# qdrant/qdrant

Hardware: AMD Instinct MI355X
Metric: QPS @ recall@10, brute-force, d=768 10M vecs, f32 cosine top-10 (higher is better)
Workload: dtype f32 (int8 prefilter + exact f32 re-score)

## Files before the change

### qdrant_amd/csrc/api_core.hip

```cpp
#include "api_internal.hpp"

namespace qmx {

static thread_local std::string g_last_error;
const std::string &last_error_text() { return g_last_error; }

void set_error(const char *fmt, ...) {
    char buf[1024];
    va_list ap;
    va_start(ap, fmt);
    vsnprintf(buf, sizeof(buf), fmt, ap);
    va_end(ap);
    g_last_error = buf;
}

int32_t hip_status(hipError_t e, const char *what, const char *file, int line) {
    set_error("HIP error %d (%s) at %s:%d: %s", (int)e, hipGetErrorString(e), file, line, what);
    (void)hipGetLastError();
    switch (e) {
        case hipErrorOutOfMemory: return QMX_ERR_OUT_OF_MEMORY;
        case hipErrorNoDevice:
        case hipErrorInvalidDevice:
        case hipErrorNoBinaryForGpu:
        case hipErrorInsufficientDriver: return QMX_ERR_NO_DEVICE;
        case hipErrorNotReady: return QMX_ERR_NOT_READY;
        case hipErrorInvalidValue: return QMX_ERR_BAD_ARG;
        default: return QMX_ERR_OTHER;
    }
}

static const char *const g_option_names[OPT_COUNT] = {"no_mfma_scan", "no_mfma16", "no_prescan", "prescan_shift", "hnsw_log_cap", "no_split_scan", "split_min_queries", "no_split256", "no_pq_pair", "no_pq_prefilter", "pq_prefilter_min_queries", "hnsw_pq_per_cu", "tq_rotate_block", "no_topk_small", "verify_max_per_query", "hnsw_pq_direct_walk", "hnsw_pq_table_build", "hnsw_no_pq_prefilter", "hnsw_no_lds_visited", "pq_lut_no_lds", "hnsw_per_cu", "hnsw_reference_heap_order", "tq_wide_min_queries", "tq_wide_high_digit", "sq_wide_min_queries", "i8_resident", "group_matrix_bytes", "debug"};
struct OptionTable {
    std::atomic<int64_t> v[OPT_COUNT];
    int64_t initial[OPT_COUNT];
    OptionTable() {
        for (int i = 0; i < OPT_COUNT; ++i) {
            char env[64] = "QMX_";
            size_t k = 4;
            for (const char *c = g_option_names[i]; *c && k + 1 < sizeof(env); ++c) env[k++] = (char)toupper((unsigned char)*c);
            env[k] = 0;
            const char *e = getenv(env);
            int64_t val = 0;
            if (e) { val = (*e >= '0' && *e <= '9') ? atoll(e) : 1; }
            if (i == OPT_PRESCAN_SHIFT && !e) val = 10;
            if (i == OPT_SPLIT_MIN_QUERIES && !e) val = 1;
            if (i == OPT_PQ_PREFILTER_MIN_QUERIES && !e) val = 4;
            if (i == OPT_TQ_WIDE_MIN_QUERIES && !e) val = 33;
            if (i == OPT_SQ_WIDE_MIN_QUERIES && !e) val = 33;
            if (i == OPT_I8_RESIDENT && !e) val = 1;
            initial[i] = val;
            v[i].store(val, std::memory_order_relaxed);
        }
    }
};
static OptionTable g_options;
int64_t option(Option o) { return g_options.v[o].load(std::memory_order_relaxed); }

static thread_local const void *g_last_kernel = nullptr;
const void *last_noted_kernel() { return g_last_kernel; }
void note_kernel(const void *host_function) { g_last_kernel = host_function; }

void clear_stale_error() {
    hipError_t e = hipGetLastError();
    if (e != hipSuccess) {
        const bool debug = option(OPT_DEBUG) != 0;
        if (debug) fprintf(stderr, "[qmx] dropped stale HIP error %d (%s) before a kernel launch\n", (int)e, hipGetErrorString(e));
    }
}

bool is_device_ptr(const void *p) {
    if (!p) return false;
    hipPointerAttribute_t attr;
    hipError_t e = hipPointerGetAttributes(&attr, p);
    if (e != hipSuccess) {
        (void)hipGetLastError();
        return false;
    }
    return attr.type == hipMemoryTypeDevice || attr.type == hipMemoryTypeManaged;
}

uint32_t elem_bytes(uint32_t dtype) {
    switch (dtype) {
        case QMX_DTYPE_F32: return 4;
        case QMX_DTYPE_F16: return 2;
        default: return 1;
    }
}



int32_t check_device(int32_t device_id, hipDeviceProp_t *prop_out) {
    int count = 0;
    hipError_t e = hipGetDeviceCount(&count);
    if (e != hipSuccess || count == 0) {
        (void)hipGetLastError();
        set_error("no HIP device visible (%s); libqdrant_amd has no CPU fallback", e == hipSuccess ? "count=0" : hipGetErrorString(e));
        return QMX_ERR_NO_DEVICE;
    }
    QMX_REQUIRE(device_id >= 0 && device_id < count, QMX_ERR_NO_DEVICE, "device %d out of range (have %d)", device_id, count);
    hipDeviceProp_t prop;
    QMX_HIP(hipGetDeviceProperties(&prop, device_id));
    QMX_REQUIRE(strncmp(prop.gcnArchName, "gfx950", 6) == 0, QMX_ERR_NO_DEVICE,
                "device %d is %s; this library ships gfx950 (MI355X) code objects only", device_id, prop.gcnArchName);
    QMX_HIP(hipSetDevice(device_id));
    if (prop_out) *prop_out = prop;
    return QMX_OK;
}

}


extern "C" {


uint32_t qmx_abi_version(void) { return 8; }

static int option_index(const char *name) {
    if (!name) return -1;
    for (int i = 0; i < OPT_COUNT; ++i)
        if (strcmp(name, g_option_names[i]) == 0) return i;
    return -1;
}
int32_t qmx_set_option(const char *name, int64_t value) {
    const int i = option_index(name);
    QMX_REQUIRE(i >= 0, QMX_ERR_BAD_ARG, "unknown option '%s'", name ? name : "(null)");
    g_options.v[i].store(value < 0 ? g_options.initial[i] : value, std::memory_order_relaxed);
    return QMX_OK;
}
int32_t qmx_get_option(const char *name, int64_t *out_value) {
    const int i = option_index(name);
    QMX_REQUIRE(i >= 0 && out_value, QMX_ERR_BAD_ARG, "unknown option '%s'", name ? name : "(null)");
    *out_value = option((Option)i);
// ... 30 lines not shown
```

### qdrant_amd/csrc/api_search.hip

```cpp
#include "api_internal.hpp"

extern "C" {

struct SearchCall {
    qmx_query *q;
    uint32_t top;
    const uint32_t *d_ids;
    uint64_t n_cand;
    qmx_scored_point *d_out;
    uint32_t *d_counts;
    const volatile uint8_t *is_stopped;
    qmx_counters *counters;
    bool timed;
    uint32_t launches;
};

static ScanArgs tile_args(const qmx_query *q, uint32_t top, uint64_t n_cand, uint32_t tile0, uint32_t nq_tile) {
    ScanArgs a;
    fill_args(q, tile0, nq_tile, a);
    a.n_cand = n_cand;
    a.top = top;
    return a;
}
static ScanArgs tile_args(const SearchCall &c, uint32_t tile0, uint32_t nq_tile) { return tile_args(c.q, c.top, c.n_cand, tile0, nq_tile); }
// ... 311 lines not shown
        QMX_TRY(launch_regroup_lists(q->stream, a.del, (const unsigned char *)q->sp_wl.p + (sq ? sqw_wlists_counts_bytes(s->num_cus) : tq4w_wlists_counts_bytes(s->num_cus)),
                                     (const uint32_t *)q->sp_wl.p, sq ? sqw_wcap() : tq4w_wcap(), grid * 8, (uint64_t *)q->sp_cand.p, (uint32_t *)q->sp_cnt.p,
                                     SPLIT_CAND_CAP, tile_ovf));
        QMX_TRY(launch_split_select(q->stream, (const uint64_t *)q->sp_cand.p, (const uint32_t *)q->sp_cnt.p, SPLIT_CAND_CAP, f.band, nq_tile, c.top, vp, tile0, tile_ovf,
                                    (uint32_t *)(plan + pl.ovf_q) + tile0, (SplitStats *)plan, tq_high ? f.wide_high : nullptr, tq_high));
        c.launches += 6;
    }
    QMX_TRY(verify_and_sort(c, vp, q->nq));
    QMX_TRY(overflow_passes(c, pl, q->nq, TQW_FQT, sq ? overflow_scan_sq : overflow_scan_tq, &c.launches));
    q->last_split = true;
    q->last_pq = false;
    q->last_fqt = TQW_FQT;
    close_counters(c, (uint64_t)q->nq * c.n_cand,
                   (uint64_t)n_tiles * c.n_cand * s->row_bytes + (uint64_t)((q->nq + MAX_QT_MFMA - 1) / MAX_QT_MFMA) * S * s->row_bytes, c.launches, q->nq);
    return QMX_OK;
}

struct SplitTiles {
    SplitPlanLayout pl;
    VerifyPool vp{};
    uint64_t S = 0;
    std::vector<std::pair<uint32_t, uint32_t>> tiles;
    SplitTiles(uint32_t nq, uint32_t fqt) : pl(nq, fqt) {}
};

static inline float split_rel_band(bool half, uint32_t dim) {
    const float acc = (float)dim * 1.1920929e-7f;
    return (half ? 9.765625e-4f + 9.5367432e-7f : 1.9073486e-6f) + acc;
}

static int32_t split_begin(const SearchCall &c, const SearchPlan &plan, SplitTiles &sp) {
    qmx_query *q = c.q;
    const qmx_segment *s = q->seg;
    QMX_TRY(q->sp_bq.reserve(split_query_bytes(s->dim)));
    QMX_TRY(q->sp_f32.reserve(SplitF32::floats * sizeof(float)));
    QMX_TRY(q->sp_cand.reserve((size_t)plan.split_qt * SPLIT_CAND_CAP * sizeof(uint64_t)));
    QMX_TRY(q->sp_cnt.reserve((size_t)SPLIT_QT_MAX * 4));
    if (s->d_rows_split) QMX_TRY(q->sp_wl.reserve(split_wlists_bytes(s->num_cus)));
    QMX_TRY(q->sp_fq.reserve((size_t)sp.pl.list_cap * q->q_stride));
    if (s->split_i8) {
        QMX_TRY(q->sp_probe.reserve((size_t)q->nq * (split_i8_probe() + 1) * 4));
        QMX_TRY(q->sp_pscores.reserve((size_t)q->nq * split_i8_probe() * 4));
    }
    return prefilter_begin(q, sp.pl, c.n_cand, s->d_rows_split ? 1 : -2, &sp.vp, &sp.S);
}

static int32_t f16_split_scan(SearchCall &c, SplitTiles &sp, const ScanArgs &a, uint32_t tile0, uint32_t nq_tile, int *tile_ovf) {
    qmx_query *q = c.q;
    const qmx_segment *s = q->seg;
    unsigned char *plan = (unsigned char *)q->sp_plan.p;
    const SplitF32 f(q->sp_f32.p);
    const float row_scale = split_row_scale(s->row_maxabs);
    const int half = s->split_half ? 1 : 0;
    const uint32_t tqt = nq_tile > SPLIT_QT ? SPLIT_QT_MAX : SPLIT_QT;
    QMX_TRY(launch_split_pack_queries(q->stream, (const float *)q->enc.p + (size_t)tile0 * s->dim, nq_tile, s->dim, f.qmax, f.qnorm, q->sp_bq.p, half, tqt));
    QMX_TRY(launch_split_thresholds(q->stream, (const uint64_t *)q->gthr.p + tile0, f.qnorm, f.qmax, nq_tile, split_rel_band(half, s->dim), s->row_norm_max, row_scale,
                                    f.scales, f.thr, f.band, tqt, (uint32_t *)q->sp_cnt.p, SPLIT_QT_MAX));
    QMX_TRY(split_stage(q, "pack + thresholds"));
    for (uint32_t phase = s->d_rows_split ? 1 : 0; phase <= (s->d_rows_split ? 2u : 0u); ++phase) {
        QMX_TIMED_SCAN(c, launch_scan_f32_split(q->stream, a, q->sp_bq.p, row_scale, f.scales, f.thr, (uint64_t *)q->sp_cand.p, (uint32_t *)q->sp_cnt.p, SPLIT_CAND_CAP,
                                                s->num_cus, s->d_rows_split, half, q->sp_wl.p, phase, tqt));
        if (s->d_rows_split)
            QMX_TRY(launch_split_regroup(q->stream, a, q->sp_wl.p, s->num_cus, (uint64_t *)q->sp_cand.p, (uint32_t *)q->sp_cnt.p, SPLIT_CAND_CAP, tile_ovf, phase, tqt));
        if (phase == 1)
            QMX_TRY(launch_split_refine(q->stream, (const uint64_t *)q->sp_cand.p, (const uint32_t *)q->sp_cnt.p, SPLIT_CAND_CAP, f.band, nq_tile, c.top, f.scales, f.thr));
    }
    QMX_TRY(split_stage(q, "split kernel"));
    QMX_TRY(launch_split_select(q->stream, (const uint64_t *)q->sp_cand.p, (const uint32_t *)q->sp_cnt.p, SPLIT_CAND_CAP, f.band, nq_tile, c.top, sp.vp, tile0, tile_ovf,
                                (uint32_t *)(plan + sp.pl.ovf_q) + tile0, (SplitStats *)plan));
    c.launches += 8;
    return QMX_OK;
}

static int32_t i8_copy_scan(SearchCall &c, SplitTiles &sp, const ScanArgs &a, uint32_t tile0, uint32_t nq_tile, int *tile_ovf) {
    qmx_query *q = c.q;
    const qmx_segment *s = q->seg;
    unsigned char *plan = (unsigned char *)q->sp_plan.p;
    const SplitF32 f(q->sp_f32.p);
    QMX_TRY(launch_split_i8_pack(q->stream, (const float *)q->enc.p + (size_t)tile0 * s->dim, nq_tile, s->dim, s->d_i8_scale, (const uint64_t *)q->gthr.p + tile0,
                                 s->d_i8_stats, s->row_norm_max, q->sp_bq.p, f.i8_qscale, f.band, f.thr, f.i8_texact, (uint32_t *)q->sp_cnt.p, SPLIT_QT_MAX));
    QMX_TRY(split_stage(q, "int8 pack"));
    const uint32_t np = split_i8_probe();
    uint32_t *probe_ids = (uint32_t *)q->sp_probe.p, *probe_cnt = probe_ids + (size_t)q->nq * np;
    const uint32_t sstride = 16;
    for (uint32_t ph = 1; ph <= 2; ++ph) {
        const uint32_t phase = ph | (sstride << 8);
        QMX_TIMED_SCAN(c, launch_scan_i8copy(q->stream, a, q->sp_bq.p, f.i8_qscale, f.thr, s->num_cus, s->d_rows_split, q->sp_wl.p, phase));
        QMX_TRY(launch_split_regroup(q->stream, a, q->sp_wl.p, s->num_cus, (uint64_t *)q->sp_cand.p, (uint32_t *)q->sp_cnt.p, SPLIT_CAND_CAP, tile_ovf, phase, SPLIT_QT));
        QMX_TRY(launch_split_i8_probe(q->stream, (const uint64_t *)q->sp_cand.p, (const uint32_t *)q->sp_cnt.p, SPLIT_CAND_CAP, f.band, nq_tile, c.top, tile_ovf,
                                      probe_ids + (size_t)tile0 * np, probe_cnt + tile0));
        const void *scan_kernel = q->last_kernel;
        PairSel psel{nullptr, np, probe_cnt};
        QMX_TRY(score_pairs_device(q, psel, probe_ids, (uint64_t)(tile0 + nq_tile) * np, (float *)q->sp_pscores.p, false));
        q->last_kernel = scan_kernel;
        QMX_TRY(launch_split_i8_bound(q->stream, (const float *)q->sp_pscores.p + (size_t)tile0 * np, probe_cnt + tile0, nq_tile, c.top, f.band, f.i8_qscale, f.thr,
                                      f.i8_texact));
    }
    QMX_TRY(split_stage(q, "int8 scan"));
    QMX_TRY(launch_split_select(q->stream, (const uint64_t *)q->sp_cand.p, (const uint32_t *)q->sp_cnt.p, SPLIT_CAND_CAP, f.band, nq_tile, c.top, sp.vp, tile0, tile_ovf,
                                (uint32_t *)(plan + sp.pl.ovf_q) + tile0, (SplitStats *)plan, f.i8_texact));
    c.launches += 13;
    return QMX_OK;
}

static int32_t split_tile(SearchCall &c, const SearchPlan &plan, SplitTiles &sp, uint32_t tile0, uint32_t nq_tile) {
    qmx_query *q = c.q;
    QMX_CHECK_CANCELLED(c.is_stopped);
    const ScanArgs a = tile_args(c, tile0, nq_tile);
    QMX_TRY(bound_enqueue(c, tile0, nq_tile, (const uint32_t *)q->sp_sample.p, sp.S, c.top, a.del, nullptr));
    QMX_TRY(split_stage(q, "prescan"));
    int *tile_ovf = (int *)((unsigned char *)q->sp_plan.p + sp.pl.tile_ovf) + sp.tiles.size();
    if (plan.route == ROUTE_I8_COPY) QMX_TRY(i8_copy_scan(c, sp, a, tile0, nq_tile, tile_ovf));
    else QMX_TRY(f16_split_scan(c, sp, a, tile0, nq_tile, tile_ovf));
    QMX_TRY(split_stage(q, "select"));
    sp.tiles.push_back({tile0, nq_tile});
    return QMX_OK;
}

static int32_t split_finish(const SearchCall &c, const SearchPlan &plan, const SplitTiles &sp) {
    qmx_query *q = c.q;
    const uint32_t first = sp.tiles.front().first, last = sp.tiles.back().first + sp.tiles.back().second;
    QMX_REQUIRE(first == 0, QMX_ERR_OTHER, "split tiles must start at query 0");
    QMX_TRY(verify_and_sort(c, sp.vp, last));
    QMX_TRY(overflow_passes(c, sp.pl, last, plan.split_fqt, overflow_scan_f32, nullptr));
    q->last_split = true;
    q->last_pq = false;
    q->last_fqt = plan.split_fqt;
    return QMX_OK;
}

static int32_t exact_tile(SearchCall &c, const SearchPlan &plan, uint32_t tile0, uint32_t nq_tile) {
    qmx_query *q = c.q;
    const qmx_segment *s = q->seg;
    const int qt = (int)pow2_ceil(nq_tile);
    for (uint32_t pass = 0; pass < plan.n_pass; ++pass) {
        QMX_CHECK_CANCELLED(c.is_stopped);
        const uint32_t off = pass * MAX_TOP_FAST;
        const uint32_t ptop = std::min<uint32_t>(MAX_TOP_FAST, c.top - off);
        ScanArgs a = tile_args(c, tile0, nq_tile);
        a.ids = c.d_ids;
        a.top = ptop;
        a.partial = (uint64_t *)q->partial.p;
        a.partial_qt = (uint32_t)qt;
        a.key_bound = pass ? (const uint64_t *)q->bounds.p : nullptr;
        const bool m16 = s->dtype == QMX_DTYPE_F32 && mfma_scan_ok(s) && mfma16_scan_ok(qt, SCAN_TOPK, a);
        const bool sqm = (s->dtype == QMX_DTYPE_SQ_U8 || s->dtype == QMX_DTYPE_TQ ? qt >= 4 : s->dtype == QMX_DTYPE_F16 && qt >= 8) && mfma_scan_ok(s);
        const bool m4 = s->dtype == QMX_DTYPE_F32 && qt >= 8 && mfma_scan_ok(s);
        const bool bqk = s->dtype == QMX_DTYPE_BQ && qt >= 4;
        if (pass == 0 && c.n_cand >= (1u << 18) && (m16 || sqm || m4 || bqk) && !option(OPT_NO_PRESCAN)) {
            const int pre_shift = (int)std::min<int64_t>(std::max<int64_t>(option(OPT_PRESCAN_SHIFT), 1), 20);
            const uint64_t pre_n = std::max<uint64_t>(c.n_cand >> pre_shift, 1u << 13) & ~(uint64_t)15;
            QMX_TRY(bound_enqueue(c, tile0, nq_tile, c.d_ids, pre_n, ptop, a.del, nullptr));
            a.gthr = (const uint64_t *)q->gthr.p + tile0;
            c.launches += 2;
        }
        uint32_t grid = (uint32_t)s->num_cus * 8;
        QMX_TIMED_SCAN(c, launch_scan(q, qt, SCAN_TOPK, a, &grid));
        QMX_TRY(launch_merge_keys(q->stream, (const uint64_t *)q->partial.p, grid, (uint32_t)qt, nq_tile, ptop, c.d_out + (size_t)tile0 * c.top, c.d_counts + tile0, c.top,
                                  off, plan.n_pass > 1 ? (uint64_t *)q->bounds.p : nullptr));
        c.launches += 2;
    }
    return QMX_OK;
}

int32_t search_enqueue(qmx_query *q, uint32_t top, const uint32_t *d_ids, uint64_t n_ids,
                              qmx_scored_point *d_out, uint32_t *d_counts, const volatile uint8_t *is_stopped,
                              qmx_counters *counters, bool timed) {
// ... 243 lines not shown
```

### qdrant_amd/csrc/common.hpp

```cpp
#pragma once
#include <hip/hip_runtime.h>
#include <hip/hip_fp16.h>
#include <stdint.h>
#include <atomic>
#include <string>

#include "../../include/qdrant_amd.h"

namespace qmx {

void set_error(const char *fmt, ...);
int32_t hip_status(hipError_t e, const char *what, const char *file, int line);
void clear_stale_error();

enum Option {
    OPT_NO_MFMA_SCAN = 0,
    OPT_NO_MFMA16,
    OPT_NO_PRESCAN,
    OPT_PRESCAN_SHIFT,
    OPT_HNSW_LOG_CAP,
    OPT_NO_SPLIT_SCAN,
    OPT_SPLIT_MIN_QUERIES,
    OPT_NO_SPLIT256,
    OPT_NO_PQ_PAIR,
    OPT_NO_PQ_PREFILTER,
    OPT_PQ_PREFILTER_MIN_QUERIES,
    OPT_HNSW_PQ_PER_CU,
    OPT_TQ_ROTATE_BLOCK,
    OPT_NO_TOPK_SMALL,
    OPT_VERIFY_MAX_PER_QUERY,
    OPT_HNSW_PQ_DIRECT_WALK,
    OPT_HNSW_PQ_TABLE_BUILD,
    OPT_HNSW_NO_PQ_PREFILTER,
    OPT_HNSW_NO_LDS_VISITED,
    OPT_PQ_LUT_NO_LDS,
    OPT_HNSW_PER_CU,
    OPT_HNSW_REFERENCE_HEAP_ORDER,
    OPT_TQ_WIDE_MIN_QUERIES,
    OPT_TQ_WIDE_HIGH_DIGIT,
    OPT_SQ_WIDE_MIN_QUERIES,
    OPT_I8_RESIDENT,
    OPT_GROUP_MATRIX_BYTES,
    OPT_DEBUG,
    OPT_COUNT
};
int64_t option(Option o);
struct DeviceOnce {
    std::atomic<uint64_t> done{0};
    int dev = 0;
    bool need() {
        if (hipGetDevice(&dev) != hipSuccess) { dev = 0; return true; }
        return dev >= 64 || !(done.load(std::memory_order_acquire) & (1ull << dev));
    }
    void mark() { if (dev < 64) done.fetch_or(1ull << dev, std::memory_order_release); }
};
void note_kernel(const void *host_function);
#define QMX_NOTE_KERNEL(fn) ::qmx::note_kernel(reinterpret_cast<const void *>(fn))

#define QMX_HIP(expr)                                                        \
    do {                                                                     \
        hipError_t e__ = (expr);                                             \
        if (e__ != hipSuccess) return ::qmx::hip_status(e__, #expr, __FILE__, __LINE__); \
    } while (0)

#define QMX_TRY(expr)                           \
    do {                                        \
        int32_t s__ = (expr);                   \
        if (s__ != QMX_OK) return s__;          \
    } while (0)

#define QMX_REQUIRE(cond, code, ...)            \
    do {                                        \
        if (!(cond)) {                          \
            ::qmx::set_error(__VA_ARGS__);      \
            return (code);                      \
        }                                       \
    } while (0)

#if defined(__HIPCC__)

constexpr int WAVE = 64;

constexpr int DPP_QUAD_XOR1 = 0xB1;
constexpr int DPP_QUAD_XOR2 = 0x4E;
constexpr int DPP_ROW_HALF_MIRROR = 0x141;
constexpr int DPP_QUAD_BCAST0 = 0x00;
constexpr int DPP_QUAD_BCAST1 = 0x55;
constexpr int DPP_QUAD_BCAST2 = 0xAA;
constexpr int DPP_QUAD_BCAST3 = 0xFF;

template <int CTRL>
__device__ __forceinline__ float dpp_f32(float v) {
    return __int_as_float(__builtin_amdgcn_update_dpp(0, __float_as_int(v), CTRL, 0xF, 0xF, true));
}
template <int CTRL>
__device__ __forceinline__ int dpp_i32(int v) {
    return __builtin_amdgcn_update_dpp(0, v, CTRL, 0xF, 0xF, true);
}

__device__ __forceinline__ uint64_t readlane_u64(uint64_t v, int lane_uniform) {
    uint32_t lo = __builtin_amdgcn_readlane((int)(uint32_t)v, lane_uniform);
    uint32_t hi = __builtin_amdgcn_readlane((int)(uint32_t)(v >> 32), lane_uniform);
    return ((uint64_t)hi << 32) | lo;
}
__device__ __forceinline__ uint64_t shfl_up1_u64(uint64_t v) {
    uint32_t lo = __shfl_up((int)(uint32_t)v, 1, 64);
    uint32_t hi = __shfl_up((int)(uint32_t)(v >> 32), 1, 64);
    return ((uint64_t)hi << 32) | lo;
}

__device__ __forceinline__ uint32_t score_to_ord(float s) {
    uint32_t b = __float_as_uint(s);
    if (s != s) return 0xFFFFFFFFu;
    return (b & 0x80000000u) ? ~b : (b | 0x80000000u);
}
__device__ __forceinline__ float ord_to_score(uint32_t o) {
    uint32_t b = (o & 0x80000000u) ? (o & 0x7FFFFFFFu) : ~o;
    return __uint_as_float(b);
}
__device__ __forceinline__ uint64_t make_key(float s, uint32_t idx) {
    return ((uint64_t)score_to_ord(s) << 32) | (uint32_t)(~idx);
}
__device__ __forceinline__ uint32_t key_idx(uint64_t k) { return ~(uint32_t)k; }
__device__ __forceinline__ float key_score(uint64_t k) { return ord_to_score((uint32_t)(k >> 32)); }
// ... 55 lines not shown
```

### qdrant_amd/csrc/scan_split.hip

```cpp
#include <type_traits>

#include "scan_common.hpp"

namespace qmx {

typedef _Float16 half8 __attribute__((ext_vector_type(8)));
typedef _Float16 half4 __attribute__((ext_vector_type(4)));
typedef float f32x4s __attribute__((ext_vector_type(4)));

constexpr int SP_BM = 256;
constexpr int SP_QT = 128;
constexpr int SP_QT_MAX = 256;
constexpr int SP_THREADS = 768;
constexpr int SP_CONSUMERS = 8;
constexpr int SP_A_UNITS = SP_BM * 2 * 4;
constexpr int SP_B_UNITS = SP_QT * 2 * 4;
constexpr int SP_BRING = 4;
constexpr int SP_LDS = (2 * SP_A_UNITS + SP_BRING * SP_B_UNITS) * 16;

__device__ __forceinline__ uint32_t sp_unit(uint32_t t, uint32_t hl, uint32_t kq, uint32_t m) { return ((t * 2 + hl) * 4 + kq) * 16 + (m ^ (2 * kq)); }

__device__ __forceinline__ void sp_split4(const f32x4s v, float scale, half4 &h, half4 &l) {
#pragma unroll
    for (int i = 0; i < 4; ++i) {
// ... 1238 lines not shown
        for (int nt = 0; nt < 4; ++nt) {
            if (!__ballot(hit[nt])) continue;
            const uint32_t q = wn * 64 + (uint32_t)nt * 16 + m_r;
#pragma unroll
            for (int mt = 0; mt < 4; ++mt) {
                int m4 = acc[mt][nt][0];
#pragma unroll
                for (int j = 1; j < 4; ++j) m4 = acc[mt][nt][j] > m4 ? acc[mt][nt][j] : m4;
                if (!__ballot(!((float)m4 < thr[nt]))) continue;
#pragma unroll
                for (int j = 0; j < 4; ++j) {
                    const float v = (float)acc[mt][nt][j];
                    const uint32_t row = row0 + (uint32_t)mt * 16 + (uint32_t)j;
                    const bool c = !(v < thr[nt]) && row < n_rows32 && q < s.nq;
                    const uint64_t hits = __ballot(c);
                    if (hits) {
                        const uint32_t at = wcount + __builtin_amdgcn_mbcnt_hi((uint32_t)(hits >> 32), __builtin_amdgcn_mbcnt_lo((uint32_t)hits, 0u));
                        if (c && at < s.wcap) {
                            const uint64_t key = make_key(v * qs[nt], row);
                            wl[at] = make_uint4((uint32_t)key, (uint32_t)(key >> 32), q, 0u);
                        }
                        wcount += (uint32_t)__builtin_popcountll(hits);
                    }
                }
            }
        }
    };
    for (uint64_t it = 0; it < my_tiles; ++it) {
        if (it) epilogue(tile_of(blockIdx.x + (it - 1) * gridDim.x));
#pragma unroll
        for (int mt = 0; mt < 4; ++mt)
#pragma unroll
            for (int nt = 0; nt < 4; ++nt) acc[mt][nt] = (i32x4s){0, 0, 0, 0};
        for (uint32_t kc = 0; kc < nch; ++kc) {
            queries_begin();
            rows_begin();
            const uint4 *ab = lds + slot * SP3_A_UNITS + a_rd;
            const uint4 *bb = b_lds + bslot * SP_B_UNITS + b_rd;
            i32x4s b0[4], b1[4];
#pragma unroll
            for (int nt = 0; nt < 4; ++nt) {
                b0[nt] = *reinterpret_cast<const i32x4s *>(bb + nt * 128);
                b1[nt] = *reinterpret_cast<const i32x4s *>(bb + nt * 128 + 64);
            }
#pragma unroll
            for (int mt = 0; mt < 4; ++mt) {
                const i32x4s a0 = *reinterpret_cast<const i32x4s *>(ab + mt * 128);
                const i32x4s a1 = *reinterpret_cast<const i32x4s *>(ab + mt * 128 + 64);
#pragma unroll
                for (int nt = 0; nt < 4; ++nt) acc[mt][nt] = __builtin_amdgcn_mfma_i32_16x16x64_i8(a1, b1[nt], acc[mt][nt], 0, 0, 0);
                if (mt == 0) queries_piece(0);
                if (mt == 1) queries_piece(1);
                if (mt == 2) { rows_piece(0); rows_piece(1); }
                if (mt == 3) { rows_piece(2); rows_piece(3); }
                __builtin_amdgcn_sched_barrier(0);
#pragma unroll
                for (int nt = 0; nt < 4; ++nt) acc[mt][nt] = __builtin_amdgcn_mfma_i32_16x16x64_i8(a0, b0[nt], acc[mt][nt], 0, 0, 0);
            }
            slot = slot + 1 == SP3_ARING ? 0 : slot + 1;
            bslot = bslot + 1 == SP8_BRING ? 0 : bslot + 1;
            asm volatile("s_waitcnt vmcnt(6)" ::: "memory");
            sp_stage_barrier();
        }
    }
    epilogue(tile_of(blockIdx.x + (my_tiles - 1) * gridDim.x));
    if (lane == 0) s.wcnt[blockIdx.x * (SP3_THREADS / 64) + (uint32_t)w] = wcount;
    asm volatile("s_waitcnt vmcnt(0)" ::: "memory");
}


constexpr uint32_t SP8R_MAX_NCH = 8;
__host__ __device__ constexpr size_t sp8r_lds_bytes(uint32_t nch) { return (size_t)nch * SP_B_UNITS * 16 + 2 * SP_QT * 4; }
template <int OFF>
__device__ __forceinline__ void sp_gload16(i32x4s &dst, const unsigned char *sbase, uint32_t voff) {
    asm volatile("global_load_dwordx4 %0, %1, %2 offset:%3 nt" : "=v"(dst) : "v"(voff), "s"(sbase), "n"(OFF) : "memory");
}
template <int I, int N, class F>
__device__ __forceinline__ void sp_static_for(F &&f) {
    if constexpr (I < N) {
        f(std::integral_constant<int, I>{});
        sp_static_for<I + 1, N>(f);
    }
}
template <int AHEAD>
__global__ __launch_bounds__(SP3_THREADS, 1) void scan_i8copy_kernel_res(const ScanArgs a, const SplitArgs s) {
    constexpr int SLOTS = AHEAD + 1, WAVES = SP3_THREADS / 64, THREADS = SP3_THREADS, MT = 2, NL = 2 * MT;
    static_assert(SP3_BM == WAVES * MT * 16, "a wave owns two row tiles of a 256-row tile");
    static_assert(NL * AHEAD <= 62, "vmcnt is six bits");
    extern __shared__ __attribute__((aligned(16))) unsigned char smem_raw[];
    uint4 *lds = reinterpret_cast<uint4 *>(smem_raw);
    const int tid = threadIdx.x, lane = tid & 63;
    const int w = __builtin_amdgcn_readfirstlane(tid >> 6);
    const uint64_t all_tiles = (a.n_cand + SP3_BM - 1) / SP3_BM;
    const uint64_t n_tiles = split_phase_tiles(all_tiles, s.phase);
    const uint32_t nch = s.nchunks;
    const uint64_t my_tiles = blockIdx.x < n_tiles ? (n_tiles - blockIdx.x + gridDim.x - 1) / gridDim.x : 0;
    const uint32_t phase = s.phase & 0xFFu, pstride = split_phase_stride(s.phase);
    auto tile_of = [&](uint64_t j) -> uint64_t { return phase == 0 ? j : phase == 1 ? j * pstride : j + j / (pstride - 1) + 1; };
    if (my_tiles == 0) {
        if (lane == 0) s.wcnt[blockIdx.x * WAVES + (uint32_t)w] = 0;
        return;
    }
    const uint32_t ws = (uint32_t)w;
    auto my_tile = [&](uint64_t i) -> uint64_t { return tile_of(blockIdx.x + i * gridDim.x); };
    float *thr_lds = reinterpret_cast<float *>(smem_raw + (size_t)nch * SP_B_UNITS * 16), *qs_lds = thr_lds + SP_QT;
#pragma unroll 4
    for (uint32_t u = (uint32_t)tid; u < nch * SP_B_UNITS; u += THREADS) lds[u] = s.bq[u];
    for (int u = tid; u < SP_QT; u += THREADS) {
        thr_lds[u] = s.thr[u];
        qs_lds[u] = s.scales[u];
    }
    __syncthreads();
    asm volatile("s_waitcnt vmcnt(0) lgkmcnt(0)" ::: "memory");
    const uint32_t kq_r = (uint32_t)lane >> 4, m_r = (uint32_t)lane & 15u;
    const uint32_t lane_unit = kq_r * 16u + (m_r ^ (2u * kq_r));
    const uint4 *const b_rd = lds + lane_unit;
    const uint32_t lane_off = lane_unit * 16u;
    auto uniform_ptr = [&](uint64_t v) {
        return reinterpret_cast<const unsigned char *>(((uint64_t)(uint32_t)__builtin_amdgcn_readfirstlane((int)(uint32_t)(v >> 32)) << 32) |
                                                       (uint32_t)__builtin_amdgcn_readfirstlane((int)(uint32_t)v));
    };
    auto load_stage = [&](uint64_t tile, uint32_t kc, i32x4s (&rc)[NL]) __attribute__((always_inline)) {
        const unsigned char *src = uniform_ptr((uint64_t)(uintptr_t)(s.rows_split + (tile * nch + kc) * SP3_A_UNITS) + ws * (NL * 1024u));
        sp_gload16<0>(rc[0], src, lane_off);
        sp_gload16<1024>(rc[1], src, lane_off);
        sp_gload16<2048>(rc[2], src, lane_off);
        sp_gload16<3072>(rc[3], src, lane_off);
    };
    i32x4s acc[MT][8];
    uint4 *const wl = s.wlist + (uint64_t)(blockIdx.x * WAVES + (uint32_t)w) * s.wcap;
    uint32_t wcount = 0;
    const uint32_t n_rows32 = (uint32_t)a.n_cand;
    auto epilogue = [&](uint64_t tile) __attribute__((always_inline)) {
        const uint32_t row0 = (uint32_t)(tile * SP3_BM) + ws * (MT * 16u) + 4 * kq_r;
        uint32_t hits8 = 0;
#pragma unroll
        for (int nt = 0; nt < 8; ++nt) {
            int mx = acc[0][nt][0];
#pragma unroll
            for (int mt = 0; mt < MT; ++mt)
#pragma unroll
                for (int j = 0; j < 4; ++j) mx = acc[mt][nt][j] > mx ? acc[mt][nt][j] : mx;
            if (!((float)mx < thr_lds[nt * 16 + (int)m_r])) hits8 |= 1u << nt;
        }
        if (!__ballot(hits8 != 0)) return;
#pragma unroll
        for (int nt = 0; nt < 8; ++nt) {
            if (!__ballot((hits8 >> nt) & 1u)) continue;
            const uint32_t q = (uint32_t)nt * 16 + m_r;
            const float th = thr_lds[q], qs = qs_lds[q];
#pragma unroll
            for (int mt = 0; mt < MT; ++mt) {
#pragma unroll
                for (int j = 0; j < 4; ++j) {
                    const float v = (float)acc[mt][nt][j];
                    const uint32_t row = row0 + (uint32_t)mt * 16 + (uint32_t)j;
                    const bool c = !(v < th) && row < n_rows32 && q < s.nq;
                    const uint64_t hits = __ballot(c);
                    if (hits) {
                        const uint32_t at = wcount + __builtin_amdgcn_mbcnt_hi((uint32_t)(hits >> 32), __builtin_amdgcn_mbcnt_lo((uint32_t)hits, 0u));
                        if (c && at < s.wcap) {
                            const uint64_t key = make_key(v * qs, row);
                            wl[at] = make_uint4((uint32_t)key, (uint32_t)(key >> 32), q, 0u);
                        }
                        wcount += (uint32_t)__builtin_popcountll(hits);
                    }
                }
            }
        }
    };
    const uint64_t n_stages = my_tiles * nch;
    uint64_t itr = 0, tile_r = my_tile(0);
    uint32_t kr = 0;
    auto advance_r = [&]() {
        if (kr + 1 < nch) ++kr;
        else if (itr + 1 < my_tiles) { kr = 0; ++itr; tile_r = my_tile(itr); }
    };
    i32x4s rc[SLOTS][NL];
    sp_static_for<0, AHEAD>([&](auto DC) __attribute__((always_inline)) {
        load_stage(tile_r, kr, rc[decltype(DC)::value]);
        advance_r();
    });
    uint64_t it = 0, tile_c = my_tile(0), tile_done = 0;
    uint32_t kc = 0;
    auto one_stage = [&](auto IC) __attribute__((always_inline)) {
        constexpr int I = decltype(IC)::value, IL = (I + AHEAD) % SLOTS;
        if (kc == 0) {
            if (it) epilogue(tile_done);
#pragma unroll
            for (int mt = 0; mt < MT; ++mt)
#pragma unroll
                for (int nt = 0; nt < 8; ++nt) acc[mt][nt] = (i32x4s){0, 0, 0, 0};
        }
        load_stage(tile_r, kr, rc[IL]);
        advance_r();
        asm volatile("s_waitcnt vmcnt(%0)" : : "n"(NL * AHEAD) : "memory");
        asm volatile("" : "+v"(rc[I][0]), "+v"(rc[I][1]), "+v"(rc[I][2]), "+v"(rc[I][3]) : : "memory");
#pragma unroll
        for (int hl = 0; hl < 2; ++hl) {
            const uint4 *bb = b_rd + kc * SP_B_UNITS + hl * 64;
            constexpr int RA = 3;
            i32x4s bv[RA + 1];
#pragma unroll
            for (int k = 0; k < RA; ++k) bv[k] = *reinterpret_cast<const i32x4s *>(bb + k * 128);
#pragma unroll
            for (int nt = 0; nt < 8; ++nt) {
                if (nt + RA < 8) bv[(nt + RA) % (RA + 1)] = *reinterpret_cast<const i32x4s *>(bb + (nt + RA) * 128);
#pragma unroll
                for (int mt = 0; mt < MT; ++mt) acc[mt][nt] = __builtin_amdgcn_mfma_i32_16x16x64_i8(rc[I][mt * 2 + hl], bv[nt % (RA + 1)], acc[mt][nt], 0, 0, 0);
                __builtin_amdgcn_sched_barrier(0);
            }
        }
        if (++kc == nch) {
            kc = 0;
            tile_done = tile_c;
            if (++it < my_tiles) tile_c = my_tile(it);
        }
    };
    for (uint64_t g = 0; g < n_stages; g += SLOTS) {
        sp_static_for<0, SLOTS>([&](auto IC) __attribute__((always_inline)) {
            if (g + decltype(IC)::value < n_stages) one_stage(IC);
        });
    }
    asm volatile("s_waitcnt vmcnt(0)" ::: "memory");
    epilogue(tile_done);
    if (lane == 0) s.wcnt[blockIdx.x * WAVES + (uint32_t)w] = wcount;
    asm volatile("s_waitcnt vmcnt(0)" ::: "memory");
}

__global__ __launch_bounds__(SEL_BLOCK) void sp_i8_probe_kernel(const uint64_t *cand, const uint32_t *cand_cnt, uint32_t cap, const float *band,
                                                                const int *tile_overflow, uint32_t top, uint32_t *probe_ids, uint32_t *probe_cnt) {
    __shared__ SelShared sel_sh;
    uint64_t (*const sh)[WAVE] = sel_sh.sh;
    SelScratch &scratch = sel_sh.scratch;
    __shared__ uint64_t sh_kth;
    __shared__ uint32_t sh_n;
    const uint32_t q = blockIdx.x;
    const uint32_t raw = cand_cnt[q];
    if (*tile_overflow || raw > cap || raw == 0 || !(band[q] < 3.0e38f)) {
        if (threadIdx.x == 0) probe_cnt[q] = 0;
        return;
    }
    const uint64_t *c = cand + (uint64_t)q * cap;
    const uint32_t k = top < SP_I8_PROBE ? top : SP_I8_PROBE;
    const uint32_t want = raw < k ? raw : k;
    if (threadIdx.x == 0) sh_n = 0;
    if (raw <= (uint32_t)SEL_SURV) block_kth_key_ranked(c, raw, want, &scratch, &sh_kth);
    else block_kth_key(c, raw, (int)want, sh, &sh_kth);
    const uint64_t kth = sh_kth;
    for (uint32_t base = 0; base < raw; base += SEL_BLOCK) {
        const uint32_t i = base + threadIdx.x;
        if (i < raw) {
            const uint64_t key = c[i];
            if (kth != 0 && key >= kth) {
                const uint32_t slot = atomicAdd(&sh_n, 1u);
                if (slot < SP_I8_PROBE) probe_ids[(uint64_t)q * SP_I8_PROBE + slot] = key_idx(key);
            }
        }
    }
    __syncthreads();
    if (threadIdx.x == 0) probe_cnt[q] = sh_n < SP_I8_PROBE ? sh_n : SP_I8_PROBE;
}
__global__ __launch_bounds__(64) void sp_i8_bound_kernel(const float *scores, uint32_t *probe_cnt, uint32_t top, const float *band, const float *qscale,
                                                         float *thr, float *t_exact) {
    const uint32_t q = blockIdx.x;
    const int lane = threadIdx.x;
    const uint32_t n = probe_cnt[q];
    const float sc = (uint32_t)lane < n ? scores[(uint64_t)q * SP_I8_PROBE + lane] : -__builtin_inff();
    uint32_t rank = 0;
    for (int j = 0; j < 64; ++j) {
        const float o = __shfl(sc, j, 64);
        rank += (o > sc || (o == sc && j < lane)) ? 1u : 0u;
    }
    if (lane == 0) probe_cnt[q] = 0;
    if (n < top || !(band[q] < 3.0e38f)) return;
    if ((uint32_t)lane < n && rank == top - 1 && sc == sc) {
        if (sc > t_exact[q]) t_exact[q] = sc;
        const float t = (sc - band[q]) / qscale[q];
        if (t > thr[q]) thr[q] = t;
    }
}

bool split_scan_ok(const ScanArgs &a) {
    return a.dim % 128 == 0 && a.dim >= 128 && a.rem_pieces == 0 && a.tail_start == a.dim && a.row_stride % 16 == 0 && a.ids == nullptr && a.top <= 64 &&
           !option(OPT_NO_SPLIT_SCAN);
}
size_t split_wlists_counts_bytes(int num_cus) { return ((size_t)num_cus * (SP3_THREADS / 64) * 4 + 255) / 256 * 256; }
size_t split_wlists_bytes(int num_cus) { return split_wlists_counts_bytes(num_cus) + (size_t)num_cus * (SP3_THREADS / 64) * SP_WCAP * 16; }
size_t split_query_bytes(uint32_t dim) { return (size_t)(dim / 32) * SP4_B_UNITS * 16; }

int32_t launch_split_row_stats(hipStream_t st, const void *rows, uint64_t row_stride, uint64_t n, uint32_t dim, uint32_t *d_stats) {
    if (n == 0) return QMX_OK;
    ::qmx::clear_stale_error();
    hipLaunchKernelGGL(sp_row_stats_kernel, dim3(2048), dim3(256), 0, st, (const unsigned char *)rows, row_stride, n, dim, d_stats);
    QMX_HIP(hipGetLastError());
    return QMX_OK;
}
float split_row_scale(float row_maxabs) {
    if (!(row_maxabs > 0.0f) || !(row_maxabs < 3.0e38f)) return 1.0f;
    int e;
    (void)frexpf(row_maxabs, &e);
    int s = 14 - e;
    s = s > 100 ? 100 : (s < -100 ? -100 : s);
    return ldexpf(1.0f, s);
}

int32_t launch_split_pack_queries(hipStream_t st, const float *d_q, uint32_t nq, uint32_t dim, float *d_qmax, float *d_qnorm, void *d_bq, int half, uint32_t qt) {
    QMX_REQUIRE(nq <= SP_QT_MAX, QMX_ERR_BAD_ARG, "split tile of %u queries", nq);
    ::qmx::clear_stale_error();
    hipLaunchKernelGGL(sp_query_stats_kernel, dim3(nq), dim3(256), 0, st, d_q, nq, dim, d_qmax, d_qnorm);
// ... 134 lines not shown
    ::qmx::clear_stale_error();
    QMX_HIP(hipMemsetAsync(d_colmax, 0, (size_t)dim * 4, st));
    QMX_HIP(hipMemsetAsync(d_colsq, 0, (size_t)dim * 4, st));
    if (n) hipLaunchKernelGGL(sp_i8_colmax_kernel, dim3(2048), dim3(256), 0, st, (const unsigned char *)rows, row_stride, n, dim, d_colmax, d_colsq);
    QMX_HIP(hipGetLastError());
    return QMX_OK;
}
float split_i8_choose_scales(const float *colmax, const float *colsq, uint64_t n, uint32_t dim, float *scale) {
    std::vector<double> s0(dim), sig(dim);
    double wmax = 0.0;
    for (uint32_t i = 0; i < dim; ++i) {
        s0[i] = colmax[i] > 1.0e-30f ? (double)colmax[i] / 127.0 : 1.0;
        sig[i] = n ? sqrt((double)colsq[i] / (double)n) : 0.0;
        if (!(sig[i] < 1.0e30)) sig[i] = 0.0;
        wmax = std::max(wmax, sig[i] * s0[i]);
    }
    auto scales_of = [&](double G, std::vector<double> &s) {
        for (uint32_t i = 0; i < dim; ++i) {
            const double w = sig[i] * s0[i];
            s[i] = (w > 0.0 && wmax / G > w && colmax[i] > 1.0e-30f) ? s0[i] * (wmax / G / w) : s0[i];
        }
    };
    auto predicted = [&](const std::vector<double> &s) {
        double vmax = 0.0, vsum = 0.0, c2 = 0.0;
        for (uint32_t i = 0; i < dim; ++i) {
            const double v = sig[i] * s[i];
            vmax = std::max(vmax, v);
            vsum += v;
            c2 += (sig[i] / s[i]) * (sig[i] / s[i]);
        }
        const double t = 3.0 * vmax / 127.0;
        if (!(t > 0.0)) return 0.0;
        double f2 = 0.0;
        for (uint32_t i = 0; i < dim; ++i) f2 += std::min(1.0 / 12.0, (sig[i] * s[i] / t) * (sig[i] * s[i] / t));
        return 0.4 * vsum + t * sqrt(c2) * sqrt(f2);
    };
    static const double grid[] = {1.0e30, 64.0, 45.0, 32.0, 23.0, 16.0, 11.0, 8.0, 5.6, 4.0, 2.8, 2.0};
    std::vector<double> s(dim), best(dim);
    double best_b = 0.0, best_g = grid[0];
    for (size_t k = 0; k < sizeof(grid) / sizeof(grid[0]); ++k) {
        scales_of(grid[k], s);
        const double b = predicted(s);
        if (k == 0 || b < best_b * 0.98) {
            best_b = b;
            best_g = grid[k];
            best = s;
        }
    }
    for (uint32_t i = 0; i < dim; ++i) {
        float f = (float)best[i];
        const float floor_s = colmax[i] > 1.0e-30f ? colmax[i] / 127.0f : 1.0f;
        scale[i] = f >= floor_s ? f : floor_s;
    }
    return best_g >= 1.0e29 ? 0.0f : (float)best_g;
}
int32_t launch_split_i8_rowstats(hipStream_t st, const void *rows, uint64_t row_stride, uint64_t n, uint32_t dim, const float *d_scale, uint32_t *d_stats) {
    QMX_REQUIRE(split_i8_dim_ok(dim), QMX_ERR_BAD_ARG, "int8 copy of dim %u", dim);
    ::qmx::clear_stale_error();
    QMX_HIP(hipMemsetAsync(d_stats, 0, 16, st));
    if (n) hipLaunchKernelGGL(sp_i8_row_stats_kernel, dim3(2048), dim3(256), 0, st, (const unsigned char *)rows, row_stride, n, dim, d_scale, d_stats);
    QMX_HIP(hipGetLastError());
    return QMX_OK;
}
int32_t launch_split_i8_copy(hipStream_t st, const void *rows, uint64_t row_stride, uint64_t n, uint32_t dim, const float *d_scale, void *d_out) {
    if (n == 0) return QMX_OK;
    ::qmx::clear_stale_error();
    hipLaunchKernelGGL(sp_i8_copy_kernel, dim3(8192), dim3(256), 0, st, (const unsigned char *)rows, row_stride, n, dim, d_scale, (uint4 *)d_out);
    QMX_HIP(hipGetLastError());
    return QMX_OK;
}
int32_t launch_split_i8_pack(hipStream_t st, const float *d_q, uint32_t nq, uint32_t dim, const float *d_scale, const uint64_t *d_gthr, const uint32_t *d_row_stats,
                             float row_norm_max, void *d_bq, float *d_qscale, float *d_band, float *d_thr, float *d_t_exact, uint32_t *d_cand_cnt, uint32_t n_cnt) {
    QMX_REQUIRE(nq <= (uint32_t)SP_QT, QMX_ERR_BAD_ARG, "int8 tile of %u queries", nq);
    ::qmx::clear_stale_error();
    hipLaunchKernelGGL(sp_i8_pack_kernel, dim3(SP_QT), dim3(256), (size_t)dim * 4, st, d_q, nq, dim, d_scale, d_gthr, d_row_stats, row_norm_max, (uint4 *)d_bq,
                       d_qscale, d_band, d_thr, d_t_exact, d_cand_cnt, n_cnt);
    QMX_HIP(hipGetLastError());
    return QMX_OK;
}
int32_t launch_scan_i8copy(hipStream_t st, const ScanArgs &a, const void *d_bq, const float *d_qscale, const float *d_thr, int num_cus, const void *d_rows_i8,
                           void *d_wlists, uint32_t phase) {
    const uint32_t nch_r = a.dim / 128;
    const bool resident = option(OPT_I8_RESIDENT) > 0 && nch_r <= SP8R_MAX_NCH;
    void (*kfn)(const ScanArgs, const SplitArgs) = resident ? scan_i8copy_kernel_res<1> : scan_i8copy_kernel;
    const size_t lds_bytes = resident ? sp8r_lds_bytes(nch_r) : (size_t)SP8_LDS;
    static thread_local DeviceOnce attr_once;
    if (attr_once.need()) {
        QMX_HIP(hipFuncSetAttribute(reinterpret_cast<const void *>(scan_i8copy_kernel), hipFuncAttributeMaxDynamicSharedMemorySize, SP8_LDS));
        QMX_HIP(hipFuncSetAttribute(reinterpret_cast<const void *>(scan_i8copy_kernel_res<1>), hipFuncAttributeMaxDynamicSharedMemorySize, (int)sp8r_lds_bytes(SP8R_MAX_NCH)));
        attr_once.mark();
    }
    QMX_REQUIRE(d_rows_i8 && d_wlists && split_i8_dim_ok(a.dim), QMX_ERR_BAD_ARG, "the int8 scan reads the int8 copy and writes per-wave candidate lists");
    SplitArgs s;
    s.rows_split = (const uint4 *)d_rows_i8;
    s.bq = (const uint4 *)d_bq;
    s.nchunks = a.dim / 128;
    s.nq = a.nq;
    s.row_scale = 1.0f;
    s.scales = d_qscale;
    s.thr = d_thr;
    s.cand = nullptr;
    s.cand_cnt = nullptr;
    s.cap = 0;
    s.wcap = SP_WCAP;
    s.wcnt = (uint32_t *)d_wlists;
    s.wlist = (uint4 *)((unsigned char *)d_wlists + split_wlists_counts_bytes(num_cus));
    s.phase = phase;
    const uint64_t n_tiles = split_phase_tiles((a.n_cand + SP3_BM - 1) / SP3_BM, phase);
    if (n_tiles == 0) return QMX_OK;
    const uint32_t grid = (uint32_t)std::max<uint64_t>(1, std::min<uint64_t>(n_tiles, (uint64_t)num_cus));
    ::qmx::clear_stale_error();
    QMX_NOTE_KERNEL(kfn);
    hipLaunchKernelGGL(kfn, dim3(grid), dim3(SP3_THREADS), lds_bytes, st, a, s);
    QMX_HIP(hipGetLastError());
    return QMX_OK;
}
int32_t launch_split_i8_probe(hipStream_t st, const uint64_t *d_cand, const uint32_t *d_cand_cnt, uint32_t cap, const float *d_band, uint32_t nq, uint32_t top,
                              const int *d_tile_overflow, uint32_t *d_probe_ids, uint32_t *d_probe_cnt) {
    ::qmx::clear_stale_error();
    hipLaunchKernelGGL(sp_i8_probe_kernel, dim3(nq), dim3(SEL_BLOCK), 0, st, d_cand, d_cand_cnt, cap, d_band, d_tile_overflow, top, d_probe_ids, d_probe_cnt);
    QMX_HIP(hipGetLastError());
    return QMX_OK;
}
int32_t launch_split_i8_bound(hipStream_t st, const float *d_scores, uint32_t *d_probe_cnt, uint32_t nq, uint32_t top, const float *d_band, const float *d_qscale,
                              float *d_thr, float *d_t_exact) {
    ::qmx::clear_stale_error();
    hipLaunchKernelGGL(sp_i8_bound_kernel, dim3(nq), dim3(64), 0, st, d_scores, d_probe_cnt, top, d_band, d_qscale, d_thr, d_t_exact);
    QMX_HIP(hipGetLastError());
    return QMX_OK;
}

}
```

Measured before the change: 98000.

## Add dense integer-threshold epilogue to the resident int8 scan phase one

Adds a dense variant of the resident int8 scan kernel for phase 1. Thresholds are pre-converted to integers so hit detection becomes integer subtracts packed into a bit mask. Hits are then emitted in a ballot loop, and the epilogue runs inline after each tile instead of being deferred into the next pipeline stage. The main loop is restructured to one stage per iteration with a rotating slot selector, which may change the load/MFMA overlap. It also exposes the sample stride as an option with the same default.

```diff
diff --git a/qdrant_amd/csrc/api_core.hip b/qdrant_amd/csrc/api_core.hip
--- a/qdrant_amd/csrc/api_core.hip
+++ b/qdrant_amd/csrc/api_core.hip
@@ -29,7 +29,7 @@
     }
 }
 
-static const char *const g_option_names[OPT_COUNT] = {"no_mfma_scan", "no_mfma16", "no_prescan", "prescan_shift", "hnsw_log_cap", "no_split_scan", "split_min_queries", "no_split256", "no_pq_pair", "no_pq_prefilter", "pq_prefilter_min_queries", "hnsw_pq_per_cu", "tq_rotate_block", "no_topk_small", "verify_max_per_query", "hnsw_pq_direct_walk", "hnsw_pq_table_build", "hnsw_no_pq_prefilter", "hnsw_no_lds_visited", "pq_lut_no_lds", "hnsw_per_cu", "hnsw_reference_heap_order", "tq_wide_min_queries", "tq_wide_high_digit", "sq_wide_min_queries", "i8_resident", "group_matrix_bytes", "debug"};
+static const char *const g_option_names[OPT_COUNT] = {"no_mfma_scan", "no_mfma16", "no_prescan", "prescan_shift", "hnsw_log_cap", "no_split_scan", "split_min_queries", "no_split256", "no_pq_pair", "no_pq_prefilter", "pq_prefilter_min_queries", "hnsw_pq_per_cu", "tq_rotate_block", "no_topk_small", "verify_max_per_query", "hnsw_pq_direct_walk", "hnsw_pq_table_build", "hnsw_no_pq_prefilter", "hnsw_no_lds_visited", "pq_lut_no_lds", "hnsw_per_cu", "hnsw_reference_heap_order", "tq_wide_min_queries", "tq_wide_high_digit", "sq_wide_min_queries", "i8_resident", "i8_dense_epilogue", "i8_sample_stride", "group_matrix_bytes", "debug"};
 struct OptionTable {
     std::atomic<int64_t> v[OPT_COUNT];
     int64_t initial[OPT_COUNT];
@@ -48,6 +48,8 @@
             if (i == OPT_TQ_WIDE_MIN_QUERIES && !e) val = 33;
             if (i == OPT_SQ_WIDE_MIN_QUERIES && !e) val = 33;
             if (i == OPT_I8_RESIDENT && !e) val = 1;
+            if (i == OPT_I8_DENSE_EPILOGUE && !e) val = 1;
+            if (i == OPT_I8_SAMPLE_STRIDE && !e) val = 16;
             initial[i] = val;
             v[i].store(val, std::memory_order_relaxed);
         }
diff --git a/qdrant_amd/csrc/api_search.hip b/qdrant_amd/csrc/api_search.hip
--- a/qdrant_amd/csrc/api_search.hip
+++ b/qdrant_amd/csrc/api_search.hip
@@ -417,7 +417,8 @@
     QMX_TRY(split_stage(q, "int8 pack"));
     const uint32_t np = split_i8_probe();
     uint32_t *probe_ids = (uint32_t *)q->sp_probe.p, *probe_cnt = probe_ids + (size_t)q->nq * np;
-    const uint32_t sstride = 16;
+    const int64_t sstride_opt = option(OPT_I8_SAMPLE_STRIDE);
+    const uint32_t sstride = sstride_opt >= 2 && sstride_opt <= 255 ? (uint32_t)sstride_opt : 16;
     for (uint32_t ph = 1; ph <= 2; ++ph) {
         const uint32_t phase = ph | (sstride << 8);
         QMX_TIMED_SCAN(c, launch_scan_i8copy(q->stream, a, q->sp_bq.p, f.i8_qscale, f.thr, s->num_cus, s->d_rows_split, q->sp_wl.p, phase));
diff --git a/qdrant_amd/csrc/common.hpp b/qdrant_amd/csrc/common.hpp
--- a/qdrant_amd/csrc/common.hpp
+++ b/qdrant_amd/csrc/common.hpp
@@ -40,6 +40,8 @@
     OPT_TQ_WIDE_HIGH_DIGIT,
     OPT_SQ_WIDE_MIN_QUERIES,
     OPT_I8_RESIDENT,
+    OPT_I8_DENSE_EPILOGUE,
+    OPT_I8_SAMPLE_STRIDE,
     OPT_GROUP_MATRIX_BYTES,
     OPT_DEBUG,
     OPT_COUNT
diff --git a/qdrant_amd/csrc/scan_split.hip b/qdrant_amd/csrc/scan_split.hip
--- a/qdrant_amd/csrc/scan_split.hip
+++ b/qdrant_amd/csrc/scan_split.hip
@@ -1344,11 +1344,19 @@
         sp_static_for<I + 1, N>(f);
     }
 }
-template <int AHEAD>
-__global__ __launch_bounds__(SP3_THREADS, 1) void scan_i8copy_kernel_res(const ScanArgs a, const SplitArgs s) {
+__device__ __forceinline__ int sp_i8_int_threshold(float th, bool live_query) {
+    constexpr int NOTHING = 1 << 30, EVERYTHING = -(1 << 30);
+    if (!live_query) return NOTHING;
+    if (!(th > -1.0e9f)) return EVERYTHING;
+    if (th > 1.0e9f) return NOTHING;
+    return (int)ceilf(th);
+}
+template <int AHEAD, bool DENSE>
+__device__ __forceinline__ void sp_i8copy_res_scan(const ScanArgs a, const SplitArgs s) {
     constexpr int SLOTS = AHEAD + 1, WAVES = SP3_THREADS / 64, THREADS = SP3_THREADS, MT = 2, NL = 2 * MT;
     static_assert(SP3_BM == WAVES * MT * 16, "a wave owns two row tiles of a 256-row tile");
     static_assert(NL * AHEAD <= 62, "vmcnt is six bits");
+    static_assert(SP8R_MAX_NCH * 128u * 128u * 128u <= (1u << 24), "the dense epilogue compares integers: every accumulator is exact in f32");
     extern __shared__ __attribute__((aligned(16))) unsigned char smem_raw[];
     uint4 *lds = reinterpret_cast<uint4 *>(smem_raw);
     const int tid = threadIdx.x, lane = tid & 63;
@@ -1369,7 +1377,8 @@
 #pragma unroll 4
     for (uint32_t u = (uint32_t)tid; u < nch * SP_B_UNITS; u += THREADS) lds[u] = s.bq[u];
     for (int u = tid; u < SP_QT; u += THREADS) {
-        thr_lds[u] = s.thr[u];
+        if constexpr (DENSE) thr_lds[u] = __int_as_float(sp_i8_int_threshold(s.thr[u], (uint32_t)u < s.nq));
+        else thr_lds[u] = s.thr[u];
         qs_lds[u] = s.scales[u];
     }
     __syncthreads();
@@ -1431,6 +1440,46 @@
             }
         }
     };
+    auto epilogue_dense = [&](uint64_t tile) __attribute__((always_inline)) {
+        static_assert(MT == 2, "a lane's hit mask is eight bits: two row tiles of four rows");
+        const uint32_t row0 = (uint32_t)(tile * SP3_BM) + ws * (MT * 16u) + 4 * kq_r;
+        uint32_t rows_there = 0xFFu;
+        if ((tile + 1) * SP3_BM > a.n_cand) {
+            rows_there = 0;
+#pragma unroll
+            for (int b = 0; b < 8; ++b) rows_there |= row0 + (uint32_t)(b >> 2) * 16 + (uint32_t)(b & 3) < n_rows32 ? 1u << b : 0u;
+        }
+        const int *const ith_lds = reinterpret_cast<const int *>(thr_lds);
+#pragma unroll
+        for (int nt = 0; nt < 8; ++nt) {
+            const uint32_t q = (uint32_t)nt * 16 + m_r;
+            const int ith = ith_lds[q];
+            uint32_t miss = 0;
+#pragma unroll
+            for (int b = 7; b >= 0; --b) miss = __builtin_amdgcn_alignbit(miss, (uint32_t)(acc[b >> 2][nt][b & 3] - ith), 31);
+            uint32_t m = ~miss & rows_there;
+            uint64_t level = __ballot(m != 0);
+            if (!level) continue;
+            const float qs = qs_lds[q];
+            do {
+                const uint32_t at = wcount + __builtin_amdgcn_mbcnt_hi((uint32_t)(level >> 32), __builtin_amdgcn_mbcnt_lo((uint32_t)level, 0u));
+                if (m != 0 && at < s.wcap) {
+                    const uint32_t h = (uint32_t)__builtin_ctz(m);
+                    const int h0 = -(int)(h & 1u), h1 = -(int)((h >> 1) & 1u), h2 = -(int)(h >> 2);
+                    auto pick = [](int mask, int if_clear, int if_set) { return (if_set & mask) | (if_clear & ~mask); };
+                    const int x = pick(h1, pick(h0, acc[0][nt][0], acc[0][nt][1]), pick(h0, acc[0][nt][2], acc[0][nt][3]));
+                    const int y = pick(h1, pick(h0, acc[1][nt][0], acc[1][nt][1]), pick(h0, acc[1][nt][2], acc[1][nt][3]));
+                    const float v = (float)pick(h2, x, y);
+                    const uint32_t row = row0 + (h >> 2) * 16 + (h & 3u);
+                    const uint64_t key = make_key(v * qs, row);
+                    wl[at] = make_uint4((uint32_t)key, (uint32_t)(key >> 32), q, 0u);
+                }
+                m &= m - 1;
+                wcount += (uint32_t)__builtin_popcountll(level);
+                level = __ballot(m != 0);
+            } while (level);
+        }
+    };
     const uint64_t n_stages = my_tiles * nch;
     uint64_t itr = 0, tile_r = my_tile(0);
     uint32_t kr = 0;
@@ -1445,14 +1494,19 @@
     });
     uint64_t it = 0, tile_c = my_tile(0), tile_done = 0;
     uint32_t kc = 0;
+    auto clear_acc = [&]() __attribute__((always_inline)) {
+#pragma unroll
+        for (int mt = 0; mt < MT; ++mt)
+#pragma unroll
+            for (int nt = 0; nt < 8; ++nt) acc[mt][nt] = (i32x4s){0, 0, 0, 0};
+    };
     auto one_stage = [&](auto IC) __attribute__((always_inline)) {
         constexpr int I = decltype(IC)::value, IL = (I + AHEAD) % SLOTS;
-        if (kc == 0) {
-            if (it) epilogue(tile_done);
-#pragma unroll
-            for (int mt = 0; mt < MT; ++mt)
-#pragma unroll
-                for (int nt = 0; nt < 8; ++nt) acc[mt][nt] = (i32x4s){0, 0, 0, 0};
+        if constexpr (!DENSE) {
+            if (kc == 0) {
+                if (it) epilogue(tile_done);
+                clear_acc();
+            }
         }
         load_stage(tile_r, kr, rc[IL]);
         advance_r();
@@ -1473,21 +1527,49 @@
                 __builtin_amdgcn_sched_barrier(0);
             }
         }
-        if (++kc == nch) {
-            kc = 0;
-            tile_done = tile_c;
-            if (++it < my_tiles) tile_c = my_tile(it);
-        }
-    };
-    for (uint64_t g = 0; g < n_stages; g += SLOTS) {
-        sp_static_for<0, SLOTS>([&](auto IC) __attribute__((always_inline)) {
-            if (g + decltype(IC)::value < n_stages) one_stage(IC);
-        });
-    }
-    asm volatile("s_waitcnt vmcnt(0)" ::: "memory");
-    epilogue(tile_done);
+        if constexpr (!DENSE) {
+            if (++kc == nch) {
+                kc = 0;
+                tile_done = tile_c;
+                if (++it < my_tiles) tile_c = my_tile(it);
+            }
+        }
+    };
+    if constexpr (DENSE) {
+        uint32_t set = 0;
+        clear_acc();
+        for (uint64_t g = 0; g < n_stages; ++g) {
+            sp_static_for<0, SLOTS>([&](auto IC) __attribute__((always_inline)) {
+                if (set == (uint32_t)decltype(IC)::value) one_stage(IC);
+            });
+            set = set + 1 == (uint32_t)SLOTS ? 0 : set + 1;
+            if (++kc == nch) {
+                kc = 0;
+                epilogue_dense(tile_c);
+                clear_acc();
+                if (++it < my_tiles) tile_c = my_tile(it);
+            }
+        }
+        asm volatile("s_waitcnt vmcnt(0)" ::: "memory");
+    } else {
+        for (uint64_t g = 0; g < n_stages; g += SLOTS) {
+            sp_static_for<0, SLOTS>([&](auto IC) __attribute__((always_inline)) {
+                if (g + decltype(IC)::value < n_stages) one_stage(IC);
+            });
+        }
+        asm volatile("s_waitcnt vmcnt(0)" ::: "memory");
+        epilogue(tile_done);
+    }
     if (lane == 0) s.wcnt[blockIdx.x * WAVES + (uint32_t)w] = wcount;
     asm volatile("s_waitcnt vmcnt(0)" ::: "memory");
+}
+template <int AHEAD>
+__global__ __launch_bounds__(SP3_THREADS, 1) void scan_i8copy_kernel_res(const ScanArgs a, const SplitArgs s) {
+    sp_i8copy_res_scan<AHEAD, false>(a, s);
+}
+template <int AHEAD>
+__global__ __launch_bounds__(SP3_THREADS, 1) void scan_i8copy_kernel_res_dense(const ScanArgs a, const SplitArgs s) {
+    sp_i8copy_res_scan<AHEAD, true>(a, s);
 }
 
 __global__ __launch_bounds__(SEL_BLOCK) void sp_i8_probe_kernel(const uint64_t *cand, const uint32_t *cand_cnt, uint32_t cap, const float *band,
@@ -1788,12 +1870,14 @@
                            void *d_wlists, uint32_t phase) {
     const uint32_t nch_r = a.dim / 128;
     const bool resident = option(OPT_I8_RESIDENT) > 0 && nch_r <= SP8R_MAX_NCH;
-    void (*kfn)(const ScanArgs, const SplitArgs) = resident ? scan_i8copy_kernel_res<1> : scan_i8copy_kernel;
+    const bool dense = resident && (phase & 0xFFu) == 1 && option(OPT_I8_DENSE_EPILOGUE) > 0;
+    void (*kfn)(const ScanArgs, const SplitArgs) = dense ? scan_i8copy_kernel_res_dense<1> : resident ? scan_i8copy_kernel_res<1> : scan_i8copy_kernel;
     const size_t lds_bytes = resident ? sp8r_lds_bytes(nch_r) : (size_t)SP8_LDS;
     static thread_local DeviceOnce attr_once;
     if (attr_once.need()) {
         QMX_HIP(hipFuncSetAttribute(reinterpret_cast<const void *>(scan_i8copy_kernel), hipFuncAttributeMaxDynamicSharedMemorySize, SP8_LDS));
         QMX_HIP(hipFuncSetAttribute(reinterpret_cast<const void *>(scan_i8copy_kernel_res<1>), hipFuncAttributeMaxDynamicSharedMemorySize, (int)sp8r_lds_bytes(SP8R_MAX_NCH)));
+        QMX_HIP(hipFuncSetAttribute(reinterpret_cast<const void *>(scan_i8copy_kernel_res_dense<1>), hipFuncAttributeMaxDynamicSharedMemorySize, (int)sp8r_lds_bytes(SP8R_MAX_NCH)));
         attr_once.mark();
     }
     QMX_REQUIRE(d_rows_i8 && d_wlists && split_i8_dim_ok(a.dim), QMX_ERR_BAD_ARG, "the int8 scan reads the int8 copy and writes per-wave candidate lists");
```

New measurement: 99040 (median of 6 runs). 1.1% higher.
